# xbpeng/DeepTerrainRL

Measured on AMD Instinct MI355X. Metric: env-steps/sec (batched rollout) dog/slopes_mixed, higher is better.
Workload: dtype f64

## Files before the change

### deepterrainrl_amd/csrc/dtrl_kernel.h

```cpp
#pragma once
#include "dtrl_types.h"
#include <cmath>

#if defined(__HIPCC__)
#include <hip/hip_runtime.h>
#define DTRL_HD __host__ __device__
#define DTRL_HD_INLINE __host__ __device__ __forceinline__
#define DTRL_HD_NOINLINE __host__ __device__ __attribute__((noinline))
#else
#define DTRL_HD
#define DTRL_HD_INLINE inline
#define DTRL_HD_NOINLINE inline
#endif

#if defined(__HIP_DEVICE_COMPILE__)
#define LANES_BEGIN { const int lane = static_cast<int>(threadIdx.x);
#define LANES_END } ::dtrl::env_sync();
#else
#define LANES_BEGIN for (int lane = 0; lane < ::dtrl::kGroup; ++lane) {
#define LANES_END }
#endif

#if defined(__HIP_DEVICE_COMPILE__) && defined(DTRL_PROFILE)
#define PROF_T0() const unsigned long long prof_t0_ = __builtin_readcyclecounter()
// ... 91 lines not shown
	real px[kMaxL], py[kMaxL], cx[kMaxL], cy[kMaxL];
	real vpx[kMaxL], vpy[kMaxL], vcx[kMaxL], vcy[kMaxL];
	real fx[kMaxL], fy[kMaxL], fn[kMaxL];
	real mcx[kMaxL], mcy[kMaxL], Io[kMaxL];
	real sfs[3][kMaxL];
	union {
		struct { real bx[kMaxL], by[kMaxL], ux[kMaxL], uy[kMaxL], gx[kMaxL], gy[kMaxL]; };
		struct { real sm[kMaxL], smx[kMaxL], smy[kMaxL], sI[kMaxL]; };
	};
	real dinv[kMaxD];
	real b[kMaxD];
	real u[kMaxD];
	int32_t R, n_pts_active;
	int32_t row_kind[kMaxRows], row_link[kMaxRows];
	int8_t row_link2[kMaxRows];
	real row_x[kMaxRows], row_y[kMaxRows], row_dx[kMaxRows], row_dy[kMaxRows], row_tgt[kMaxRows];
	uint16_t row_id[kMaxRows];
	real wv[kMaxRows], rinv[kMaxRows];
	real dl;
	union {
		real Z[kMaxRows + 1][kZStride];
		struct {
			real z0_[kZStride];
			real basis[kMaxD][4];
			real tau_g[kMaxD];
			real kpv[kMaxD], kdv[kMaxD], kdm[kMaxD], perr[kMaxD], verr[kMaxD];
		};
	};
	real red[8];
	int32_t flag_update_action, flag_new_cycle, flag_misc;
	int32_t cost;
#if defined(DTRL_PROFILE)
	unsigned long long prof[kProfMax];
#endif
};
struct WSRef : WSBase {
	real H[kMaxD][kMaxD + 1];
	union {
		real A[kMaxRows][kMaxRows + 1];
		struct {
			real pt_x[kMaxPts], pt_y[kMaxPts], pt_depth[kMaxPts], pt_nx[kMaxPts], pt_ny[kMaxPts];
			int32_t pt_active[kMaxPts];
		};
	};
};
constexpr int kPackedA = kMaxRows * (kMaxRows + 1) / 2;
constexpr int kMassTab = kMaxL * (kMaxDepth + 2);
struct WSFast : WSBase {
	real Apk[kPackedA > kMassTab ? kPackedA : kMassTab];
};


DTRL_HD_INLINE real fmadd(real a, real b, real c) { return __builtin_fma(a, b, c); }
DTRL_HD_INLINE void sincos_r(real x, real* s, real* c)
{
#if defined(DTRL_REAL_F32)
	sincosf(x, s, c);
#else
	sincos(x, s, c);
#endif
}
#if defined(__HIP_DEVICE_COMPILE__)
typedef real v4r_t __attribute__((ext_vector_type(4)));
__device__ __forceinline__ v4r_t mfma_16x16x4(real a, real b, v4r_t acc)
{
#if defined(DTRL_REAL_F32)
	return __builtin_amdgcn_mfma_f32_16x16x4f32(a, b, acc, 0, 0, 0);
#else
	return __builtin_amdgcn_mfma_f64_16x16x4f64(a, b, acc, 0, 0, 0);
#endif
}
__device__ __forceinline__ constexpr int mfma_row(int r, int g)
{
#if defined(DTRL_REAL_F32)
	return 4 * g + r;
#else
	return 4 * r + g;
#endif
}
#endif
DTRL_HD_INLINE real fast_recip(real x)
{
#if defined(__HIP_DEVICE_COMPILE__)
	real r = __builtin_amdgcn_rcp(x);
	r = __builtin_fma(__builtin_fma(-x, r, 1.0), r, r);
	r = __builtin_fma(__builtin_fma(-x, r, 1.0), r, r);
	return r;
#else
	return 1.0 / x;
#endif
}
DTRL_HD_INLINE real fast_rsqrt(real x)
{
#if defined(__HIP_DEVICE_COMPILE__)
	real r = __builtin_amdgcn_rsq(x);
	const real hx = 0.5 * x;
	r = __builtin_fma(__builtin_fma(-hx * r, r, 0.5), r, r);
	r = __builtin_fma(__builtin_fma(-hx * r, r, 0.5), r, r);
	return r;
#else
	return 1.0 / sqrt(x);
#endif
}

DTRL_HD_INLINE real clamp_turn_rate(real v, int dof, real h)
{
	if (dof < 2) return v;
	const real vmax = kMaxTurnPerSubstep / h;
	return v > vmax ? vmax : (v < -vmax ? -vmax : v);
}
DTRL_HD inline real wrap_pi(real a)
{
	const real pi = 3.14159265358979323846, two_pi = 6.283185307179586476925286766559;
	real r = fmod(a + pi, two_pi);
	if (r < 0) r += two_pi;
	return r - pi;
}

DTRL_HD inline uint64_t rng_mix(uint64_t x)
{
	x += 0x9E3779B97F4A7C15ULL;
	x = (x ^ (x >> 30)) * 0xBF58476D1CE4E5B9ULL;
	x = (x ^ (x >> 27)) * 0x94D049BB133111EBULL;
	return x ^ (x >> 31);
}
struct Rng {
	uint64_t key; uint64_t* ctr;
	DTRL_HD real uniform() { uint64_t z = rng_mix(key + (*ctr) * 0xD1342543DE82EF95ULL); ++(*ctr); return static_cast<real>(z >> 11) * (1.0 / 9007199254740992.0); }
	DTRL_HD real uniform(real mn, real mx) { return mn + uniform() * (mx - mn); }
	DTRL_HD int rand_int(int mn, int mx) { if (mn == mx) return mn; int r = mn + static_cast<int>(uniform() * (mx - mn)); return r >= mx ? mx - 1 : r; }
	DTRL_HD bool flip() { return uniform() < 0.5; }
	DTRL_HD real normal(real mean, real stdev)
	{
		real u1 = 1.0 - uniform(), u2 = uniform();
		return mean + stdev * sqrt(-2.0 * log(u1)) * cos(6.283185307179586476925286766559 * u2);
	}
};
DTRL_HD inline Rng make_rng(const RunParams& rp, int env, uint64_t* ctr)
{
	Rng r; r.key = rng_mix(rp.rng_seed ^ rng_mix(static_cast<uint64_t>(rp.env_id_base + env))); r.ctr = ctr; return r;
}

struct GroundHdr { real mx0, o0, o1, sc0, sc1; int w0, w1; };
DTRL_HD_INLINE GroundHdr ground_header(const GroundRec& g)
{
	GroundHdr h;
	h.mx0 = g.max_x[0]; h.w0 = g.w[0]; h.w1 = g.w[1];
	h.o0 = g.origin_x[0]; h.o1 = g.origin_x[1]; h.sc0 = g.scale_x[0]; h.sc1 = g.scale_x[1];
	return h;
}
DTRL_HD_INLINE real sample_ground(const GroundRec& g, const GroundHdr& gh, real x, real* slope, int* oi, int* oj, int* oseg)
{
	const real mx0 = gh.mx0;
	const int w0 = gh.w0, w1 = gh.w1;
	const real o0 = gh.o0, o1 = gh.o1, sc0 = gh.sc0, sc1 = gh.sc1;
	const int seg = (x >= mx0) ? 1 : 0;
	const int w = seg ? w1 : w0;
	const real scale = seg ? sc1 : sc0;
	const real tol = 0.0001;
	real c = x - (seg ? o1 : o0);
	c /= scale;
	c += ((w - 1) * 0.5);
	if (c > -tol && c < w - 1 + tol) { c = c < 0.0 ? 0.0 : (c > w - 1.0 ? w - 1.0 : c); }
	c = !(c > 0.0) ? 0.0 : (c > w - 1.0 ? w - 1.0 : c);
	int i = static_cast<int>(c);
	int j = (i + 1 < w - 1) ? i + 1 : w - 1;
	real lerp = c - i;
	const real inv_run = fast_recip(scale * ((j - i) > 0 ? (j - i) : 1));
	real a = g.data[seg][i];
	real b = g.data[seg][j];
	if (slope) *slope = (j == i) ? 0.0 : (b - a) * inv_run;
	if (oi) *oi = i;
	if (oj) *oj = j;
	if (oseg) *oseg = seg;
	return (1 - lerp) * a + lerp * b;
}
DTRL_HD_INLINE real sample_ground(const GroundRec& g, real x, real* slope, int* oi, int* oj, int* oseg)
{
	const GroundHdr gh = ground_header(g);
	return sample_ground(g, gh, x, slope, oi, oj, oseg);
}

static_assert(kMaxDepth % 4 == 0, "path rows are read as 32-bit words");
template <class W>
DTRL_HD_INLINE uint32_t path_word(const W& ws, int j, int t)
{
#if defined(__HIP_DEVICE_COMPILE__)
	return reinterpret_cast<const uint32_t*>(&ws.M.path[j][0])[t];
#else
	uint32_t w; __builtin_memcpy(&w, &ws.M.path[j][4 * t], 4); return w;
#endif
}
template <class W>
DTRL_HD inline void kin_dyn_terms(W& ws)
{
	PROF_T0();
	LANES_BEGIN
	if (lane < ws.M.L) {
		const int j = lane;
		const int dep = ws.M.depth[j];
		real phi = 0, w = 0;
		const uint32_t pw[kMaxDepth / 4] = {path_word(ws, j, 0), path_word(ws, j, 1), path_word(ws, j, 2)};
#pragma unroll
		for (int k = 0; k < kMaxDepth; ++k) {
			const int a = (k <= dep) ? static_cast<int>((pw[k / 4] >> (8 * (k % 4))) & 0xffu) : 0;
			const real qa = ws.st.q[a + 2], wa = ws.st.qd[a + 2];
			const real on = (k <= dep) ? 1.0 : 0.0;
			phi = fmadd(qa, on, phi); w = fmadd(wa, on, w);
		}
		ws.phi[j] = phi; ws.w[j] = w;
		real s, c; sincos_r(phi, &s, &c);
		ws.cs[j] = c; ws.sn[j] = s;
	}
	LANES_END
	PROF_ADD(ws, kProfP1);
	LANES_BEGIN
	if (lane < ws.M.L) {
		const int j = lane;
		const int pa = ws.M.parent[j];
		real rx = 0, ry = 0, ux = 0, uy = 0, gx = 0, gy = 0;
		if (pa >= 0) {
			const real c = ws.cs[pa], s = ws.sn[pa], wp = ws.w[pa];
			rx = c * ws.M.attach[j][0] - s * ws.M.attach[j][1];
			ry = s * ws.M.attach[j][0] + c * ws.M.attach[j][1];
			ux = -(wp * ry); uy = wp * rx;
			const real w2 = wp * wp;
			gx = -(w2 * rx); gy = -(w2 * ry);
		}
// ... 1192 lines not shown
				else transition_state(ws, next);
			}
		} else {
			if ((state == stBackStance || state == stFrontStance) && ws.st.phase >= 1) advance = true;
			int trans_contact = (state == stExtend) ? jFinger : ((state == stGather) ? jToe : -1);
			if (trans_contact >= 0 && in_contact(ws, trans_contact)) advance = true;
			if (advance) {
				int next = ws.st.first_cycle ? stBackStance : ((state == stGather) ? stInvalid : state + 1);
				bool end_step = (next == stInvalid) || ws.st.first_cycle;
				if (end_step) do_update = 1; else transition_state(ws, next);
			}
		}
		ws.flag_update_action = do_update;
	}
	LANES_END
	PROF_ADD_SINCE(ws, kProfC_Fsm, pc_t); pc_t = PROF_NOW();
	if (__builtin_expect(ws.flag_update_action != 0, 0)) {
		PROF_T0();
		update_action<Ext>(ws, gm, rp, buf, g, env);
		PROF_ADD(ws, kProfAction);
		if (Ext) { if (ws.st.ext_park == kExtAwaiting) return; }
		LANES_BEGIN
		if (lane == 0) ws.st.first_cycle = 0;
		LANES_END
	}
	}
	LANES_BEGIN
	if (lane == 0) {
		real sx = 0, m = 0;
		for (int j = 0; j < L; ++j) { sx += ws.M.mass[j] * ws.vcx[j]; m += ws.M.mass[j]; }
		real com_vx = sx / m;
		if (raptor) {
			const int sh = stance_joint(ws, 0), st_toe = stance_joint(ws, 3);
			if (raptor_active_effector(ws, st_toe)) ws.st.pd_active_bits &= ~(1u << sh); else ws.st.pd_active_bits |= (1u << sh);
			real cv = ws.st.params[rmpCv], cd = ws.st.params[rmpCd];
			const bool first_half = ws.st.state == rstContact || ws.st.state == rstDown;
			cd = first_half ? 0 : cd; cv = first_half ? cv : 0;
			real com[2]; calc_com(ws, com);
			real d_theta = cd * (com[0] - (ws.st.q[0] + ws.cx[st_toe])) + cv * com_vx;
			ws.st.pd_target[swing_joint(ws, 0)] = ws.st.params[rmpMax + ws.st.state * rspMax + rspSwingHip] + d_theta;
		} else {
			const int joints[2] = {jHip, jShoulder}, effs[2] = {jToe, jFinger}, prm[2] = {spHip, spShoulder};
			for (int k = 0; k < 2; ++k) if (!in_contact(ws, effs[k])) {
				real default_theta = ws.st.params[mpMax + ws.st.state * spMax + prm[k]];
				ws.st.pd_target[joints[k]] = default_theta + com_vx * ws.st.params[mpCv];
			}
		}
	}
	LANES_END
	PROF_ADD_SINCE(ws, kProfC_Feedback, pc_t); pc_t = PROF_NOW();
	LANES_BEGIN
	if (lane < D) {
		const int i = lane;
		real kp = 0, kd = 0, kdm = 0, pe = 0, ve = 0;
		if (i >= 3) {
			const int j = i - 2;
			kdm = gm.kd[j];
			if ((ws.st.pd_active_bits >> j) & 1u) { kp = gm.kp[j]; kd = kdm; }
			real theta;
			if (gm.use_world[j]) {
				theta = wrap_pi(ws.phi[j] + gm.body_theta[j]);
				if (theta <= real(-2.0943951023931954923084289221863)) theta += real(6.283185307179586476925286766559);
			} else {
				theta = wrap_pi(ws.st.q[i] + gm.ref_theta[j]) - gm.ref_theta[j];
			}
			pe = ws.st.pd_target[j] - theta;
			ve = 0 - ws.st.qd[i];
		}
		ws.kpv[i] = kp; ws.kdv[i] = kd; ws.kdm[i] = kdm; ws.perr[i] = pe; ws.verr[i] = ve;
		ws.u[i] = kp * (pe - dt * ws.st.qd[i]) + kd * ve - quirk_bias(ws, i);
	}
	LANES_END
	PROF_ADD_SINCE(ws, kProfC_PdSetup, pc_t); pc_t = PROF_NOW();
	Path::pd_solve(ws, dt);
	PROF_ADD_SINCE(ws, kProfC_PdSolve, pc_t); pc_t = PROF_NOW();
	LANES_BEGIN
	if (lane < D) { const int i = lane; ws.tau_g[i] = 0; ws.st.tau_ctrl[i] = ws.kpv[i] * (ws.perr[i] - dt * ws.st.qd[i]) + ws.kdv[i] * (ws.verr[i] - dt * ws.u[i]); }
	LANES_END
	const int eff0 = raptor ? int(rRightToe) : int(jToe), eff1 = raptor ? int(rLeftToe) : int(jFinger);
	const bool sup0 = raptor ? raptor_active_effector(ws, eff0) : in_contact(ws, eff0);
	const bool sup1 = raptor ? raptor_active_effector(ws, eff1) : in_contact(ws, eff1);
	if (gm.enable_grav_comp && (sup0 || sup1)) {
		LANES_BEGIN
		if (lane < D) {
			const int d = lane;
			real tg;
			const real gy = kGravityY;
			if (d == 0) tg = 0;
			else if (d == 1) tg = -(ws.sm[0] * gy);
			else { const int l = d - 2; tg = -((ws.smx[l] - ws.sm[l] * ws.px[l]) * gy); }
			ws.tau_g[d] = tg;
			for (int e = 0; e < 2; ++e) {
				const int jid = e ? eff1 : eff0;
				real b0 = 0, b1 = 0;
				bool on_path = (d < 3) || ((ws.M.sub_mask[d - 2] >> jid) & 1u);
				if ((e ? sup1 : sup0) && on_path) {
					real pos[2]; effector_pos(ws, gm, jid, pos);
					const real fy[2] = {0, 1}, fxv[2] = {1, 0};
					b0 = jt_force(ws, d, pos, fy); b1 = jt_force(ws, d, pos, fxv);
				}
				ws.basis[d][e * 2 + 0] = b0; ws.basis[d][e * 2 + 1] = b1;
			}
		}
		LANES_END
		LANES_BEGIN
		if (lane == 0) {
			const real Wd[3] = {1, 1, 1}, Wr[3] = {0.0001, 0.0001, 1};
			real x[4];
			solve_ls4(ws.basis, ws.tau_g, raptor ? Wr : Wd, x);
			for (int k = 0; k < 4; ++k) ws.red[k] = x[k];
		}
		LANES_END
		LANES_BEGIN
		if (lane < D && (raptor || lane >= 3)) {
			const int d = lane;
			real s = 0; for (int k = 0; k < 4; ++k) s += ws.basis[d][k] * ws.red[k];
			ws.st.tau_ctrl[d] += ws.tau_g[d] - s;
		}
		LANES_END
	}
	PROF_ADD_SINCE(ws, kProfC_Grav, pc_t); pc_t = PROF_NOW();
	if (raptor) {
		LANES_BEGIN
// ... 363 lines not shown
```

### deepterrainrl_amd/csrc/dtrl_kernel_fast.h

```cpp
#pragma once
#include "dtrl_kernel.h"
#include "dtrl_topo.h"
#include <type_traits>

#if defined(__HIP_DEVICE_COMPILE__)

#if !DTRL_WAVE_SYNC
#error "dtrl_kernel_fast.h: the register-resident path is ONE wavefront per env by construction (v_readlane broadcasts, ballots, and LDS read-then-write sequences such as warm_match_fast() that rely on a wave's LDS operations completing in issue order). -DDTRL_WAVE_SYNC=0 builds the lane-phase reference path only (ADVICE r5)"
#endif

namespace dtrl {

__device__ __forceinline__ int lane_id() { return static_cast<int>(threadIdx.x); }
__device__ __forceinline__ int opaque_lane()
{
	int lane = static_cast<int>(threadIdx.x);
	asm volatile("" : "+v"(lane));
	return lane;
}
#if defined(DTRL_REAL_F32)
#define DTRL_VFMA "v_fma_f32"
#define DTRL_VMOV "v_mov_b32"
#else
#define DTRL_VFMA "v_fma_f64"
#define DTRL_VMOV "v_mov_b64"
#endif
__device__ __forceinline__ real bcast(real v, int src)
{
#if defined(DTRL_REAL_F32)
	return __int_as_float(__builtin_amdgcn_readlane(__float_as_int(v), src));
#else
	int lo = __builtin_amdgcn_readlane(__double2loint(v), src);
	int hi = __builtin_amdgcn_readlane(__double2hiint(v), src);
	return __hiloint2double(hi, lo);
#endif
}

template <int D>
__device__ __forceinline__ void mass_row(WSFast& ws, real (&h)[D])
{
	constexpr int Lk = D - 2;
	constexpr int kTab = Lk * (Lk + 5) / 2;
	constexpr int kFill = (kTab + 1) & ~1;
	static_assert(kFill <= static_cast<int>(sizeof(ws.Apk) / sizeof(real)), "mass table does not fit the packed-matrix storage");
	const int d = static_cast<int>(threadIdx.x);
	const int l = d >= 2 ? d - 2 : 0;
	const bool hinge = d >= 2 && d < D;
	real* T = ws.Apk;
	{
		struct alignas(2 * sizeof(real)) real2 { real x, y; };
		real2* T2 = reinterpret_cast<real2*>(T);
		const real2 z2 = {0.0, 0.0};
#pragma unroll
		for (int e = 0; e < (kFill / 2 + kGroup - 1) / kGroup; ++e) if (d + e * kGroup < kFill / 2) T2[d + e * kGroup] = z2;
	}
	env_sync();
	if (hinge) {
		const int base = l * (l + 5) / 2;
		const real m = ws.sm[l], mx = ws.smx[l], my = ws.smy[l];
		T[base] = -(my - m * ws.py[l]);
		T[base + 1] = (mx - m * ws.px[l]);
	}
	const int n_pairs = ws.M.n_pairs;
#pragma unroll 2
	for (int e = lane_id(); e < n_pairs; e += kGroup) {
		const int pl = ws.M.pair_l[e], pk = ws.M.pair_k[e];
		const int a = ws.M.path[pl][pk];
		const real m = ws.sm[pl], mx = ws.smx[pl], my = ws.smy[pl], I = ws.sI[pl];
		const real plx = ws.px[pl], ply = ws.py[pl];
		const real pax = ws.px[a], pay = ws.py[a];
		T[pl * (pl + 5) / 2 + 2 + a] = I - ((plx + pax) * mx + (ply + pay) * my) + m * (plx * pax + ply * pay);
	}
// ... 104 lines not shown
		fnma_lanes_lt<k>(z, h[k], zk);
	});
	return z;
}
template <class Topo>
constexpr int first_update_col(int i)
{
	for (int k = Topo::L + 1; k > i; --k) if (dof_coupled<Topo>(i, k)) return k;
	return 0;
}
template <class Topo, int kAhead = 1>
__device__ __forceinline__ void usolve_rows(WSFast& ws, int R)
{
	constexpr int D = Topo::L + 2;
	const int lane = static_cast<int>(threadIdx.x);
	if (lane > R) return;
	real* z = ws.Z[lane];
	const real* U = ws.Apk;
	real acc[D], u[D * (D - 1) / 2];
	auto fetch = [&](auto kc) {
		constexpr int k = decltype(kc)::value;
		static_for<0, k>([&](auto ic) {
			constexpr int i = decltype(ic)::value;
			if constexpr (dof_coupled<Topo>(i, k)) u[k * (k - 1) / 2 + i] = U[k * (k - 1) / 2 + i];
			if constexpr (first_update_col<Topo>(i) == k) acc[i] = z[i];
		});
		if constexpr (first_update_col<Topo>(k) == 0) acc[k] = z[k];
	};
	static_for_down<D - kAhead, D>(fetch);
	static_for_down<1, D>([&](auto kc) {
		constexpr int k = decltype(kc)::value;
		__builtin_amdgcn_sched_barrier(0);
		if constexpr (k - kAhead >= 1) fetch(std::integral_constant<int, k - kAhead>{});
		const real zk = acc[k];
		if constexpr (first_update_col<Topo>(k) != 0) z[k] = zk;
		static_for_down<0, k>([&](auto ic) {
			constexpr int i = decltype(ic)::value;
			if constexpr (dof_coupled<Topo>(i, k)) acc[i] = fmadd(-u[k * (k - 1) / 2 + i], zk, acc[i]);
		});
	});
	z[0] = acc[0];
}
template <int D>
__device__ __forceinline__ real utsolve_regs(const real (&h)[D], real u)
{
	static_for<0, D - 1>([&](auto kc) {
		constexpr int k = decltype(kc)::value;
		const real uk = bcast(u, k);
		fnma_lanes_ge<k + 1>(u, h[k], uk);
	});
	return u;
}

static_assert((kMaxPts + kGroup - 1) / kGroup == 3, "written for 3 sample points per lane");
struct ContactPts { PtVal p0, p1, p2; unsigned long long m0, m1, m2;  unsigned long long f0, f1, f2;  };
__device__ __forceinline__ unsigned link_field(unsigned long long m0, unsigned long long m1, unsigned long long m2, int link)
{
	const int b = link * kPtsPerLink, word = b >> 6, off = b & 63;
	unsigned long long lo = m0, hi = m1;
	if (word == 1) { lo = m1; hi = m2; }
	if (word == 2) { lo = m2; hi = 0ull; }
	unsigned long long bits = lo >> off;
	if (off + kPtsPerLink > 64) bits |= hi << (64 - off);
	return static_cast<unsigned>(bits & ((1ull << kPtsPerLink) - 1ull));
}
constexpr real kNoPoint = -1.0e30;
__device__ __noinline__ unsigned link_cap_drop_mask(WSFast& ws, real d0, real d1, real d2)
{
	const int lane = opaque_lane();
	const int npts = ws.M.L * kPtsPerLink;
	real* S = ws.Apk;
	if (lane < npts) S[lane] = d0;
	if (lane + kGroup < npts) S[lane + kGroup] = d1;
	if (lane + 2 * kGroup < npts) S[lane + 2 * kGroup] = d2;
	env_sync();
	auto over = [&](real d, int pt) -> unsigned {
		if (!(d > kNoPoint)) return 0u;
		const int base = (pt / kPtsPerLink) * kPtsPerLink;
		int rank = 0;
		for (int k = 0; k < kPtsPerLink; ++k) { const int o = base + k; const real od = S[o]; rank += (o != pt && (od > d || (od == d && o < pt))) ? 1 : 0; }
		return rank >= kMaxPtsPerLink ? 1u : 0u;
	};
	const unsigned m = over(d0, lane) | (over(d1, lane + kGroup) << 1) | (over(d2, lane + 2 * kGroup) << 2);
	env_sync();
	return m;
}
template <bool kFlags>
__device__ __forceinline__ ContactPts eval_points(WSFast& ws, const DevModel& gm, const GroundRec& g)
{
	const int lane = opaque_lane();
	const int npts = ws.M.L * kPtsPerLink;
	ContactPts c;
	PtVal z; z.x = 0; z.y = 0; z.depth = 0; z.nx = 0; z.ny = 0; z.active = 0; z.near = 0;
	c.p0 = z; c.p1 = z; c.p2 = z;
	if (lane < npts) c.p0 = contact_point_eval<kFlags>(ws, gm, g, lane);
	if (lane + kGroup < npts) c.p1 = contact_point_eval<kFlags>(ws, gm, g, lane + kGroup);
	if (lane + 2 * kGroup < npts) c.p2 = contact_point_eval<kFlags>(ws, gm, g, lane + 2 * kGroup);
	c.f0 = 0; c.f1 = 0; c.f2 = 0;
	if (kFlags) { c.f0 = __ballot(c.p0.near); c.f1 = __ballot(c.p1.near); c.f2 = __ballot(c.p2.near); }
	c.m0 = __ballot(c.p0.active); c.m1 = __ballot(c.p1.active); c.m2 = __ballot(c.p2.active);
	if ((c.m0 | c.m1 | c.m2) != 0ull) {
		const int many = (lane < ws.M.L) && __popc(link_field(c.m0, c.m1, c.m2, lane)) > kMaxPtsPerLink;
		if (__builtin_expect(__ballot(many) != 0ull, 0)) {
			const unsigned drop = link_cap_drop_mask(ws, c.p0.active ? c.p0.depth : kNoPoint, c.p1.active ? c.p1.depth : kNoPoint, c.p2.active ? c.p2.depth : kNoPoint);
			if (drop & 1u) c.p0.active = 0;
			if (drop & 2u) c.p1.active = 0;
			if (drop & 4u) c.p2.active = 0;
			c.m0 = __ballot(c.p0.active); c.m1 = __ballot(c.p1.active); c.m2 = __ballot(c.p2.active);
		}
	}
	return c;
}
__device__ __noinline__ unsigned row_cap_drop_mask(WSFast& ws, real d0, real d1, real d2, int cap)
{
	const int lane = opaque_lane();
	const int npts = ws.M.L * kPtsPerLink;
	real* S = ws.Apk;
	if (lane < npts) S[lane] = d0;
	if (lane + kGroup < npts) S[lane + kGroup] = d1;
	if (lane + 2 * kGroup < npts) S[lane + 2 * kGroup] = d2;
	env_sync();
	auto over = [&](real d, int pt) -> unsigned {
		if (!(d > kNoPoint)) return 0u;
		int rank = 0;
		for (int o = 0; o < npts; ++o) { const real od = S[o]; rank += (o != pt && (od > d || (od == d && o < pt))) ? 1 : 0; }
		return rank >= cap ? 1u : 0u;
	};
	const unsigned m = over(d0, lane) | (over(d1, lane + kGroup) << 1) | (over(d2, lane + 2 * kGroup) << 2);
	env_sync();
	return m;
}
__device__ __forceinline__ unsigned long long pairs_in_reach(const WSFast& ws)
{
	const int lane = static_cast<int>(threadIdx.x);
	return __ballot(lane < ws.M.n_cpairs && pair_in_reach(ws, lane));
}
constexpr int kPairCands = 2 * kPtsPerLink, kPairSlots = kGroup / kPairCands;
__device__ __noinline__ int append_pair_rows_fast(WSFast& ws, const DevModel& gm, int R, unsigned long long reach)
{
	const int lane = opaque_lane();
	const unsigned long long below = (lane == 0) ? 0ull : (~0ull >> (64 - lane));
	const int slot = lane / kPairCands, cand = lane - slot * kPairCands;
	while (reach != 0ull && R + 2 <= kMaxRows) {
		int mypr = -1;
#pragma unroll
		for (int sidx = 0; sidx < kPairSlots; ++sidx) {
			if (reach != 0ull) { const int pr = __ffsll(static_cast<long long>(reach)) - 1; reach &= reach - 1ull; if (slot == sidx) mypr = pr; }
		}
		int P = 0, Q = 0, k = 0;
		PairHit hit; hit.active = 0; hit.depth = 0; hit.x = 0; hit.y = 0; hit.nx = 0; hit.ny = 0;
		if (mypr >= 0) { pair_candidate(ws.M.cp_a[mypr], ws.M.cp_b[mypr], cand, &P, &Q, &k); hit = pair_point_eval(ws, gm, P, Q, k); }
		const unsigned long long am = __ballot(hit.active);
		if (am == 0ull) continue;
		int keep = hit.active;
		const int mine_cnt = __popcll((am >> (slot * kPairCands)) & ((1ull << kPairCands) - 1ull));
		if (__builtin_expect(__ballot(lane < kPairSlots * kPairCands && mine_cnt > kMaxPtsPerPair) != 0ull, 0)) {
			real* S = ws.Apk;
			S[lane] = hit.active ? hit.depth : -1.0;
			env_sync();
			if (hit.active) {
				int rank = 0;
				for (int o = 0; o < kPairCands; ++o) { const real od = S[slot * kPairCands + o]; rank += (o != cand && od > 0 && (od > hit.depth || (od == hit.depth && o < cand))) ? 1 : 0; }
				keep = rank < kMaxPtsPerPair;
			}
			env_sync();
		}
		const unsigned long long km = __ballot(keep);
		const int room = (kMaxRows - R) / 2;
		const int idx = __popcll(km & below);
		if (keep && idx < room) {
			const int Rw = R + 2 * idx;
			ws.row_kind[Rw] = 1; ws.row_link[Rw] = P; ws.row_link2[Rw] = static_cast<int8_t>(Q); ws.row_x[Rw] = hit.x; ws.row_y[Rw] = hit.y;
			ws.row_dx[Rw] = hit.nx; ws.row_dy[Rw] = hit.ny; ws.row_tgt[Rw] = 0;
			ws.row_id[Rw] = pair_row_id(mypr, cand, 0); ws.row_id[Rw + 1] = pair_row_id(mypr, cand, 1);
			ws.row_kind[Rw + 1] = 2; ws.row_link[Rw + 1] = P; ws.row_link2[Rw + 1] = static_cast<int8_t>(Q); ws.row_x[Rw + 1] = hit.x; ws.row_y[Rw + 1] = hit.y;
			ws.row_dx[Rw + 1] = hit.ny; ws.row_dy[Rw + 1] = -hit.nx; ws.row_tgt[Rw + 1] = 0;
		}
		int n = __popcll(km); if (n > room) n = room;
		R += 2 * n;
	}
	return R;
}
__device__ __forceinline__ void contact_bits_fast(WSFast& ws, unsigned long long m0, unsigned long long m1, unsigned long long m2)
{
	const int lane = static_cast<int>(threadIdx.x);
	int any = 0;
	if (lane < ws.M.L) any = link_field(m0, m1, m2, lane) != 0u;
	const unsigned long long lm = __ballot(any);
	if (lane == 0) ws.st.contact_bits = static_cast<uint32_t>(lm);
}
__device__ __forceinline__ void detect_contacts_fast(WSFast& ws, const DevModel& gm, const GroundRec& g)
{
	const ContactPts c = eval_points<true>(ws, gm, g);
	contact_bits_fast(ws, c.f0, c.f1, c.f2);
	env_sync();
}
__device__ __forceinline__ void emit_contact_rows(WSFast& ws, const PtVal& p, int pt, int rank, int cap, int R0, real inv_h)
{
	if (p.active && rank < cap) {
		const int R = R0 + 2 * rank;
		const int j = pt / kPtsPerLink;
		ws.row_kind[R] = 1; ws.row_link[R] = j; ws.row_link2[R] = -1; ws.row_x[R] = p.x; ws.row_y[R] = p.y;
		ws.row_dx[R] = p.nx; ws.row_dy[R] = p.ny; ws.row_tgt[R] = normal_row_target(p.depth, inv_h);
		ws.row_id[R] = ground_row_id(pt, 0); ws.row_id[R + 1] = ground_row_id(pt, 1);
		ws.row_kind[R + 1] = 2; ws.row_link[R + 1] = j; ws.row_link2[R + 1] = -1; ws.row_x[R + 1] = p.x; ws.row_y[R + 1] = p.y;
		ws.row_dx[R + 1] = p.ny; ws.row_dy[R + 1] = -p.nx; ws.row_tgt[R + 1] = 0;
	}
}
__device__ __forceinline__ void build_rows_fast(WSFast& ws, const DevModel& gm, const ContactPts& c_in, real h)
{
	ContactPts c = c_in;
	const int lane = opaque_lane();
	const unsigned long long below = (lane == 0) ? 0ull : (~0ull >> (64 - lane));
	const real inv_h = 1.0 / h;
	int lim = 0; real tgt = 0;
	if (lane >= 1 && lane < ws.M.L && !(ws.M.lim_lo[lane] > ws.M.lim_hi[lane])) {
		const real th = ws.st.q[lane + 2];
		if (th <= ws.M.lim_lo[lane] + kLimitSlop) { lim = 1; tgt = kLimitErp * fmax(ws.M.lim_lo[lane] - th, 0.0) * inv_h; }
		else if (th >= ws.M.lim_hi[lane] - kLimitSlop) { lim = -1; tgt = kLimitErp * fmax(th - ws.M.lim_hi[lane], 0.0) * inv_h; }
	}
	const unsigned long long ml = __ballot(lim != 0);
	const int rl = __popcll(ml & below);
	int R0 = __popcll(ml); if (R0 > kMaxRows) R0 = kMaxRows;
	if (lim != 0 && rl < kMaxRows) { ws.row_kind[rl] = 0; ws.row_link[rl] = lane; ws.row_link2[rl] = -1; ws.row_dx[rl] = lim; ws.row_tgt[rl] = tgt; ws.row_id[rl] = kNoRowId; }
	const int cap = (kMaxRows - R0) / 2;
	if (__builtin_expect(__popcll(c.m0) + __popcll(c.m1) + __popcll(c.m2) > cap, 0)) {
		const unsigned drop = row_cap_drop_mask(ws, c.p0.active ? c.p0.depth : kNoPoint, c.p1.active ? c.p1.depth : kNoPoint, c.p2.active ? c.p2.depth : kNoPoint, cap);
		if (drop & 1u) c.p0.active = 0;
		if (drop & 2u) c.p1.active = 0;
		if (drop & 4u) c.p2.active = 0;
		c.m0 = __ballot(c.p0.active); c.m1 = __ballot(c.p1.active); c.m2 = __ballot(c.p2.active);
	}
	const int n0 = __popcll(c.m0), n1 = __popcll(c.m1), n2 = __popcll(c.m2);
	emit_contact_rows(ws, c.p0, lane, __popcll(c.m0 & below), cap, R0, inv_h);
	emit_contact_rows(ws, c.p1, lane + kGroup, n0 + __popcll(c.m1 & below), cap, R0, inv_h);
	emit_contact_rows(ws, c.p2, lane + 2 * kGroup, n0 + n1 + __popcll(c.m2 & below), cap, R0, inv_h);
	int nc = n0 + n1 + n2; if (nc > cap) nc = cap;
	int R = R0 + 2 * nc;
	const unsigned long long reach = pairs_in_reach(ws);
	if (__builtin_expect(reach != 0ull, 0)) R = append_pair_rows_fast(ws, gm, R, reach);
	if (lane == 0) ws.R = R;
	env_sync();
}

template <int D>
__device__ __forceinline__ void build_delassus_fast(WSFast& ws, real h, real dinv_mine)
{
	const int lane = static_cast<int>(threadIdx.x);
	const int R = ws.R;
	const int n_ent = R * (R + 1) / 2;
	if (R < 16) {
		typedef v4r_t v4d_t;
		const int g = lane >> 4, c = lane & 15;
		real jv = 0;
		if (lane < R) {
			const int sw = lane;
			if (ws.row_kind[sw] == 0) jv = ws.row_dx[sw] * ws.st.qd[ws.row_link[sw] + 2];
			else jv = row_point_jv(ws, sw);
		}
		const int zrow = c <= R ? c : 0;
		v4d_t acc = {0, 0, 0, 0};
#pragma unroll
		for (int s4 = 0; s4 < (D + 3) / 4; ++s4) {
			const int k = 4 * s4 + g;
			const bool live = k < D;
			const real z = ws.Z[zrow][live ? k : 0], dk = ws.dinv[live ? k : 0];
			const real b = live ? z : 0.0;
			const real a = live ? z * dk : 0.0;
			acc = mfma_16x16x4(a, b, acc);
		}
#pragma unroll
		for (int r = 0; r < 4; ++r) {
			const int i = mfma_row(r, g);
			if (i < R && c <= i) ws.Apk[i * (i + 1) / 2 + c] = acc[r];
			if (i < R && c == R) ws.wv[i] = acc[r];
		}
		env_sync();
		if (lane < R) ws.wv[lane] = jv + h * ws.wv[lane] - ws.row_tgt[lane];
		env_sync();
		return;
	}
	const real* di = ws.dinv;
	auto entry_rows = [](int e, int& s, int& r) {
		s = static_cast<int>((sqrtf(8.0f * e + 1.0f) - 1.0f) * 0.5f);
		while (s * (s + 1) / 2 > e) --s;
		while ((s + 1) * (s + 2) / 2 <= e) ++s;
		r = e - s * (s + 1) / 2;
	};
	{
// ... 159 lines not shown
				pgs_rows_sweep<0, kPgsRegRows>(a, w, lam, rinv, tang, (static_cast<unsigned long long>(rows_hi) << 32) | rows_lo, lane, last);
			}
		}
		if (mine) ws.st.ws_lam[lane] = lam;
		env_sync();
		return;
	}
	const int tri = lane * (lane + 1) / 2;
	if (any_l0) for (int r = 0; r < R; ++r) if ((nz_l0 >> r) & 1ull) { const int mx = lane > r ? lane : r, mn = lane < r ? lane : r; w = fmadd(ws.Apk[mine ? mx * (mx + 1) / 2 + mn : 0], bcast(lam, r), w); }
	real a_nx = mine ? ws.Apk[tri] : 0.0;
	const unsigned long long actR = act & ((R < 64) ? ((1ull << R) - 1ull) : ~0ull);
	if (warm) {
		const unsigned long long pass0 = actR & ~tmask, pass1 = actR & tmask;
		for (int it = 0; it < kPgsIters; ++it) {
			for (int r = 0; r < R; ++r) {
				const real a_sr = a_nx;
				const int rn = (r + 1 < R) ? r + 1 : 0;
				{ const int mx = lane > rn ? lane : rn, mn = lane < rn ? lane : rn; a_nx = ws.Apk[mine ? mx * (mx + 1) / 2 + mn : 0]; }
				if (!((pass0 >> r) & 1ull)) continue;
				pgs_row_step<kPgsRowNormal>(w, lam, rinv, a_sr, r, lane, false, 0.0, 0.0);
			}
			const real ln = wave_shr1(lam);
			const real lim = kMu * ln;
			const unsigned long long rows = pass1 & __ballot(tang && ln > kHoldEps);
			for (int r = 0; r < R; ++r) {
				const real a_sr = a_nx;
				const int rn = (r + 1 < R) ? r + 1 : 0;
				{ const int mx = lane > rn ? lane : rn, mn = lane < rn ? lane : rn; a_nx = ws.Apk[mine ? mx * (mx + 1) / 2 + mn : 0]; }
				if (!((rows >> r) & 1ull)) continue;
				pgs_row_step<kPgsRowFriction>(w, lam, rinv, a_sr, r, lane, false, -lim, lim);
			}
		}
	} else {
		for (int it = 0; it < kPgsIters; ++it) {
			for (int r = 0; r < R; ++r) {
				const real a_sr = a_nx;
				const int rn = (r + 1 < R) ? r + 1 : 0;
				{ const int mx = lane > rn ? lane : rn, mn = lane < rn ? lane : rn; a_nx = ws.Apk[mine ? mx * (mx + 1) / 2 + mn : 0]; }
				if (!((act >> r) & 1ull)) continue;
				pgs_row_step<kPgsRowGeneric>(w, lam, rinv, a_sr, r, lane, tang, 0.0, 0.0);
			}
		}
	}
	if (mine) ws.st.ws_lam[lane] = lam;
	env_sync();
}

#if defined(DTRL_PROFILE)
__device__ __forceinline__ int prof_row_bucket(int R) { return R == 0 ? 0 : (R <= 6 ? 1 : (R <= 12 ? 2 : (R <= 18 ? 3 : 4))); }
#endif
template <class Topo>
struct FastPath {
	static constexpr int D = Topo::L + 2;
	static __device__ void substep(WSFast& ws, const DevModel& gm, const GroundRec& g, real h, bool kin_valid)
	{
		const int lane = static_cast<int>(threadIdx.x);
#if defined(DTRL_PROFILE)
		const unsigned long long prof_sub_t0 = __builtin_readcyclecounter();
#endif
		if (!kin_valid) { PROF_T0(); kin_dyn_terms(ws); PROF_ADD(ws, kProfFK); }
		const int rows_ready = kin_valid ? ws.n_pts_active : -1;
		if (rows_ready >= 0) {
			if (lane == 0) { ws.R = rows_ready; ws.n_pts_active = -1; }
			env_sync();
		} else {
			ContactPts cp;
			{ PROF_T0(); cp = eval_points<false>(ws, gm, g); PROF_ADD(ws, kProfDetect); }
			{ PROF_T0(); build_rows_fast(ws, gm, cp, h); PROF_ADD(ws, kProfRows); }
		}
		{ PROF_T0(); warm_match_fast(ws); PROF_ADD(ws, kProfRows); }
		real hrow[D];
		{ PROF_T0(); mass_row<D>(ws, hrow); PROF_ADD(ws, kProfMass); }
		real dinv;
		{ PROF_T0(); dinv = factorize_regs<Topo>(ws, hrow); PROF_ADD(ws, kProfFact); }
		const int R = ws.R;
		if (lane == 0) ws.cost += 8 + R;
		{
			PROF_T0();
			const bool hinge = lane >= 2 && lane < D;
			const real mypx = hinge ? ws.px[lane - 2] : 0.0, mypy = hinge ? ws.py[lane - 2] : 0.0;
			const uint32_t mysub = hinge ? ws.M.sub_mask[lane - 2] : 0u;
			real rhs0 = (lane < D) ? (ws.st.tau[lane] - ws.b[lane]) : 0.0;
			if (__builtin_expect(ws.st.pert_on != 0, 0)) { if (lane < D) rhs0 += perturb_gen_force(ws, lane); }
			auto rhs_of = [&](int r) -> real {
				if (r >= R) return rhs0;
				const int kind = ws.row_kind[r], link = ws.row_link[r];
				const real dx = ws.row_dx[r];
				if (kind == 0) return (lane == link + 2) ? dx : 0.0;
				const real dy = ws.row_dy[r], x = ws.row_x[r], y = ws.row_y[r];
				const int link2 = ws.row_link2[r];
				if (lane == 0) return link2 < 0 ? dx : 0.0;
				if (lane == 1) return link2 < 0 ? dy : 0.0;
				const int on = static_cast<int>((mysub >> link) & 1u) - (link2 < 0 ? 0 : static_cast<int>((mysub >> link2) & 1u));
				if (on == 0) return 0.0;
				const real jr = dx * (-(y - mypy)) + dy * (x - mypx);
				return on > 0 ? jr : -jr;
			};
			if (R < 1) {
				if (0 <= R) {
					const real z = usolve_regs<D>(hrow, rhs_of(0));
					if (lane < D) ws.Z[0][lane] = z;
				}
			} else {
				for (int r = 0; r <= R; ++r) { const real v = rhs_of(r); if (lane < D) ws.Z[r][lane] = v; }
				env_sync();
				usolve_rows<Topo>(ws, R);
			}
			if (lane < D) ws.dinv[lane] = dinv;
			env_sync();
			PROF_ADD(ws, kProfFsub);
#if defined(DTRL_PROFILE)
			PROF_ADD(ws, kProfFsubR0 + prof_row_bucket(R));
#endif
		}
		if (R > 0) {
			{ PROF_T0(); build_delassus_fast<D>(ws, h, dinv); PROF_ADD(ws, kProfDelassus); }
			{ PROF_T0(); pgs_solve_fast<Topo::kPgsRegRows>(ws); PROF_ADD(ws, kProfPgs); }
		}
		{
			PROF_T0();
			real u = 0;
			if (lane < D) {
				real s = h * ws.Z[R][lane];
				for (int r = 0; r < R; ++r) s = fmadd(ws.Z[r][lane], ws.st.ws_lam[r], s);
				u = s * dinv;
			}
			u = utsolve_regs<D>(hrow, u);
			if (lane < D) { const real v = clamp_turn_rate(ws.st.qd[lane] + u, lane, h); ws.st.qd[lane] = v; ws.st.q[lane] += h * v; }
			env_sync();
			PROF_ADD(ws, kProfFinish);
		}
#if defined(DTRL_PROFILE)
		if (threadIdx.x == 0) { ws.prof[kProfRowsSum] += R; ws.prof[kProfSubsteps] += 1; const int bk = prof_row_bucket(R); ws.prof[kProfR0 + bk] += 1; ws.prof[kProfT0 + bk] += __builtin_readcyclecounter() - prof_sub_t0; }
#endif
	}
	static __device__ void pd_solve(WSFast& ws, real dt)
	{
		const int lane = static_cast<int>(threadIdx.x);
		real hrow[D];
		mass_row<D>(ws, hrow);
		const real add = (lane < D) ? dt * ws.kdm[lane] : 0.0;
#pragma unroll
		for (int k = 0; k < D; ++k) if (lane == k) hrow[k] += add;
		const real dinv = factorize_regs<Topo>(ws, hrow);
		real z = (lane < D) ? ws.u[lane] : 0.0;
		z = usolve_regs<D>(hrow, z);
		real u = z * dinv;
		u = utsolve_regs<D>(hrow, u);
		env_sync();
		if (lane < D) ws.u[lane] = u;
		if (lane == 0) ws.R = 0;
		env_sync();
	}
	static __device__ void contacts(WSFast& ws, const DevModel& gm, const GroundRec& g, real h)
	{
		const ContactPts cp = eval_points<true>(ws, gm, g);
		contact_bits_fast(ws, cp.f0, cp.f1, cp.f2);
		build_rows_fast(ws, gm, cp, h);
		if (threadIdx.x == 0) ws.n_pts_active = ws.R;
		env_sync();
	}
};

}
#endif
```

Baseline: 20.00 million.

## Specialize contact point evaluation on link count and batch ground loads

Contact point evaluation is templated on the topology's link count, so the number of sample points per lane is a compile-time constant and unused point slots, ballots and cap-drop branches are removed. Per-point link data and ground cells are gathered in separate batched phases so the memory loads can be issued together before the arithmetic, with asm barriers pinning the loaded values. The PD setup is also rewritten branch-free using a clamped index and selects instead of divergent branches. The risks are higher register pressure from holding all points' values at once and some extra work on lanes that are not hinges.

```diff
diff --git a/deepterrainrl_amd/csrc/dtrl_kernel.h b/deepterrainrl_amd/csrc/dtrl_kernel.h
--- a/deepterrainrl_amd/csrc/dtrl_kernel.h
+++ b/deepterrainrl_amd/csrc/dtrl_kernel.h
@@ -167,6 +167,13 @@
 
 
 DTRL_HD_INLINE real fmadd(real a, real b, real c) { return __builtin_fma(a, b, c); }
+DTRL_HD_INLINE int opaque_index(int v)
+{
+#if defined(__HIP_DEVICE_COMPILE__)
+	asm volatile("" : "+v"(v));
+#endif
+	return v;
+}
 DTRL_HD_INLINE void sincos_r(real x, real* s, real* c)
 {
 #if defined(DTRL_REAL_F32)
@@ -264,7 +271,8 @@
 	h.o0 = g.origin_x[0]; h.o1 = g.origin_x[1]; h.sc0 = g.scale_x[0]; h.sc1 = g.scale_x[1];
 	return h;
 }
-DTRL_HD_INLINE real sample_ground(const GroundRec& g, const GroundHdr& gh, real x, real* slope, int* oi, int* oj, int* oseg)
+struct GroundCell { int seg, i, j; real lerp, inv_run; };
+DTRL_HD_INLINE GroundCell ground_cell(const GroundHdr& gh, real x)
 {
 	const real mx0 = gh.mx0;
 	const int w0 = gh.w0, w1 = gh.w1;
@@ -278,17 +286,28 @@
 	c += ((w - 1) * 0.5);
 	if (c > -tol && c < w - 1 + tol) { c = c < 0.0 ? 0.0 : (c > w - 1.0 ? w - 1.0 : c); }
 	c = !(c > 0.0) ? 0.0 : (c > w - 1.0 ? w - 1.0 : c);
-	int i = static_cast<int>(c);
-	int j = (i + 1 < w - 1) ? i + 1 : w - 1;
-	real lerp = c - i;
-	const real inv_run = fast_recip(scale * ((j - i) > 0 ? (j - i) : 1));
-	real a = g.data[seg][i];
-	real b = g.data[seg][j];
-	if (slope) *slope = (j == i) ? 0.0 : (b - a) * inv_run;
-	if (oi) *oi = i;
-	if (oj) *oj = j;
-	if (oseg) *oseg = seg;
-	return (1 - lerp) * a + lerp * b;
+	GroundCell k;
+	k.seg = seg;
+	k.i = static_cast<int>(c);
+	k.j = (k.i + 1 < w - 1) ? k.i + 1 : w - 1;
+	k.lerp = c - k.i;
+	k.inv_run = fast_recip(scale * ((k.j - k.i) > 0 ? (k.j - k.i) : 1));
+	return k;
+}
+DTRL_HD_INLINE real ground_height(const GroundCell& k, real a, real b, real* slope)
+{
+	if (slope) *slope = (k.j == k.i) ? 0.0 : (b - a) * k.inv_run;
+	return (1 - k.lerp) * a + k.lerp * b;
+}
+DTRL_HD_INLINE real sample_ground(const GroundRec& g, const GroundHdr& gh, real x, real* slope, int* oi, int* oj, int* oseg)
+{
+	const GroundCell k = ground_cell(gh, x);
+	real a = g.data[k.seg][k.i];
+	real b = g.data[k.seg][k.j];
+	if (oi) *oi = k.i;
+	if (oj) *oj = k.j;
+	if (oseg) *oseg = k.seg;
+	return ground_height(k, a, b, slope);
 }
 DTRL_HD_INLINE real sample_ground(const GroundRec& g, real x, real* slope, int* oi, int* oj, int* oseg)
 {
@@ -1587,23 +1606,20 @@
 	LANES_BEGIN
 	if (lane < D) {
 		const int i = lane;
-		real kp = 0, kd = 0, kdm = 0, pe = 0, ve = 0;
-		if (i >= 3) {
-			const int j = i - 2;
-			kdm = gm.kd[j];
-			if ((ws.st.pd_active_bits >> j) & 1u) { kp = gm.kp[j]; kd = kdm; }
-			real theta;
-			if (gm.use_world[j]) {
-				theta = wrap_pi(ws.phi[j] + gm.body_theta[j]);
-				if (theta <= real(-2.0943951023931954923084289221863)) theta += real(6.283185307179586476925286766559);
-			} else {
-				theta = wrap_pi(ws.st.q[i] + gm.ref_theta[j]) - gm.ref_theta[j];
-			}
-			pe = ws.st.pd_target[j] - theta;
-			ve = 0 - ws.st.qd[i];
-		}
+		const bool hinge = i >= 3;
+		const int j = opaque_index(hinge ? i - 2 : 1);
+		const real c_kd = gm.kd[j], c_kp = gm.kp[j], c_body = gm.body_theta[j], c_ref = gm.ref_theta[j];
+		const bool world = gm.use_world[j] != 0;
+		const real qd_i = ws.st.qd[i];
+		const bool active = ((ws.st.pd_active_bits >> j) & 1u) != 0;
+		const real kdm = hinge ? c_kd : 0;
+		const real kp = (hinge && active) ? c_kp : 0, kd = (hinge && active) ? c_kd : 0;
+		const real wr = wrap_pi(world ? ws.phi[j] + c_body : ws.st.q[i] + c_ref);
+		const real theta = world ? ((wr <= real(-2.0943951023931954923084289221863)) ? wr + real(6.283185307179586476925286766559) : wr) : wr - c_ref;
+		const real pe = hinge ? ws.st.pd_target[j] - theta : 0;
+		const real ve = hinge ? 0 - qd_i : 0;
 		ws.kpv[i] = kp; ws.kdv[i] = kd; ws.kdm[i] = kdm; ws.perr[i] = pe; ws.verr[i] = ve;
-		ws.u[i] = kp * (pe - dt * ws.st.qd[i]) + kd * ve - quirk_bias(ws, i);
+		ws.u[i] = kp * (pe - dt * qd_i) + kd * ve - quirk_bias(ws, i);
 	}
 	LANES_END
 	PROF_ADD_SINCE(ws, kProfC_PdSetup, pc_t); pc_t = PROF_NOW();
diff --git a/deepterrainrl_amd/csrc/dtrl_kernel_fast.h b/deepterrainrl_amd/csrc/dtrl_kernel_fast.h
--- a/deepterrainrl_amd/csrc/dtrl_kernel_fast.h
+++ b/deepterrainrl_amd/csrc/dtrl_kernel_fast.h
@@ -18,6 +18,8 @@
 	asm volatile("" : "+v"(lane));
 	return lane;
 }
+template <class T>
+__device__ __forceinline__ void pin_loaded(T& v) { asm volatile("" : "+v"(v)); }
 #if defined(DTRL_REAL_F32)
 #define DTRL_VFMA "v_fma_f32"
 #define DTRL_VMOV "v_mov_b32"
@@ -228,27 +230,30 @@
 	return u;
 }
 
-static_assert((kMaxPts + kGroup - 1) / kGroup == 3, "written for 3 sample points per lane");
+static_assert((kMaxPts + kGroup - 1) / kGroup == 3, "written for up to 3 sample points per lane");
+constexpr int pts_per_lane(int L) { return (L * kPtsPerLink + kGroup - 1) / kGroup; }
 struct ContactPts { PtVal p0, p1, p2; unsigned long long m0, m1, m2;  unsigned long long f0, f1, f2;  };
+template <int NP>
 __device__ __forceinline__ unsigned link_field(unsigned long long m0, unsigned long long m1, unsigned long long m2, int link)
 {
 	const int b = link * kPtsPerLink, word = b >> 6, off = b & 63;
-	unsigned long long lo = m0, hi = m1;
-	if (word == 1) { lo = m1; hi = m2; }
-	if (word == 2) { lo = m2; hi = 0ull; }
+	unsigned long long lo = m0, hi = NP > 1 ? m1 : 0ull;
+	if constexpr (NP > 1) if (word == 1) { lo = m1; hi = NP > 2 ? m2 : 0ull; }
+	if constexpr (NP > 2) if (word == 2) { lo = m2; hi = 0ull; }
 	unsigned long long bits = lo >> off;
 	if (off + kPtsPerLink > 64) bits |= hi << (64 - off);
 	return static_cast<unsigned>(bits & ((1ull << kPtsPerLink) - 1ull));
 }
 constexpr real kNoPoint = -1.0e30;
+template <int NP>
 __device__ __noinline__ unsigned link_cap_drop_mask(WSFast& ws, real d0, real d1, real d2)
 {
 	const int lane = opaque_lane();
 	const int npts = ws.M.L * kPtsPerLink;
 	real* S = ws.Apk;
 	if (lane < npts) S[lane] = d0;
-	if (lane + kGroup < npts) S[lane + kGroup] = d1;
-	if (lane + 2 * kGroup < npts) S[lane + 2 * kGroup] = d2;
+	if constexpr (NP > 1) if (lane + kGroup < npts) S[lane + kGroup] = d1;
+	if constexpr (NP > 2) if (lane + 2 * kGroup < npts) S[lane + 2 * kGroup] = d2;
 	env_sync();
 	auto over = [&](real d, int pt) -> unsigned {
 		if (!(d > kNoPoint)) return 0u;
@@ -257,44 +262,99 @@
 		for (int k = 0; k < kPtsPerLink; ++k) { const int o = base + k; const real od = S[o]; rank += (o != pt && (od > d || (od == d && o < pt))) ? 1 : 0; }
 		return rank >= kMaxPtsPerLink ? 1u : 0u;
 	};
-	const unsigned m = over(d0, lane) | (over(d1, lane + kGroup) << 1) | (over(d2, lane + 2 * kGroup) << 2);
+	unsigned m = over(d0, lane);
+	if constexpr (NP > 1) m |= over(d1, lane + kGroup) << 1;
+	if constexpr (NP > 2) m |= over(d2, lane + 2 * kGroup) << 2;
 	env_sync();
 	return m;
 }
-template <bool kFlags>
+template <int L, bool kFlags>
 __device__ __forceinline__ ContactPts eval_points(WSFast& ws, const DevModel& gm, const GroundRec& g)
 {
+	constexpr int NP = pts_per_lane(L), npts = L * kPtsPerLink;
 	const int lane = opaque_lane();
-	const int npts = ws.M.L * kPtsPerLink;
+	const GroundHdr gh = ground_header(g);
+	const real q0 = ws.st.q[0], q1 = ws.st.q[1];
+	const real tol = kFlags ? gm.contact_tol : real(0);
+	bool have[NP]; int col[NP]; real lx[NP], ly[NP], margin[NP], brk[NP], cs[NP], sn[NP], px[NP], py[NP];
+	static_for<0, NP>([&](auto ec) {
+		constexpr int e = decltype(ec)::value;
+		const int pt = lane + e * kGroup;
+		have[e] = (e + 1) * kGroup <= npts || pt < npts;
+		const int ptc = ((e + 1) * kGroup <= npts || pt < npts) ? pt : npts - 1;
+		const int j = ptc / kPtsPerLink;
+		col[e] = ws.M.col[j];
+		cs[e] = ws.cs[j]; sn[e] = ws.sn[j]; px[e] = ws.px[j]; py[e] = ws.py[j];
+		const real* lp = &gm.pt_ground[0][0][0] + 2 * ptc;
+		lx[e] = lp[0]; ly[e] = lp[1];
+		margin[e] = gm.link_margin[j]; brk[e] = gm.link_brk[j];
+	});
+	static_for<0, NP>([&](auto ec) {
+		constexpr int e = decltype(ec)::value;
+		pin_loaded(col[e]); pin_loaded(lx[e]); pin_loaded(ly[e]); pin_loaded(margin[e]); pin_loaded(brk[e]);
+	});
+	real x[NP], y[NP]; GroundCell cell[NP];
+	static_for<0, NP>([&](auto ec) {
+		constexpr int e = decltype(ec)::value;
+		x[e] = px[e] + cs[e] * lx[e] - sn[e] * ly[e];
+		y[e] = py[e] + sn[e] * lx[e] + cs[e] * ly[e];
+		cell[e] = ground_cell(gh, q0 + x[e]);
+	});
+	real ha[NP], hb[NP];
+	static_for<0, NP>([&](auto ec) {
+		constexpr int e = decltype(ec)::value;
+		ha[e] = g.data[cell[e].seg][cell[e].i];
+		hb[e] = g.data[cell[e].seg][cell[e].j];
+	});
+	PtVal r[3];
+	static_for<0, 3>([&](auto ec) {
+		constexpr int e = decltype(ec)::value;
+		r[e].x = 0; r[e].y = 0; r[e].depth = 0; r[e].nx = 0; r[e].ny = 0; r[e].active = 0; r[e].near = 0;
+		if constexpr (e < NP) {
+			real slope;
+			const real h = ground_height(cell[e], ha[e], hb[e], &slope);
+			const real gap = h - (q1 + y[e]);
+			const bool in_reach = kFlags || (gap + (margin[e] + brk[e]) * (1.0 + fabs(slope)) > 0);
+			const real inv = fast_rsqrt(1.0 + slope * slope);
+			const real depth = fmadd(gap, inv, margin[e]);
+			const bool live = have[e] & (col[e] != 0);
+			if (kFlags) r[e].near = (live & (depth >= -tol)) ? 1 : 0;
+			r[e].active = (live & in_reach & (depth > -brk[e])) ? 1 : 0;
+			r[e].nx = -slope * inv; r[e].ny = inv;
+			r[e].depth = depth;
+			r[e].x = x[e]; r[e].y = y[e];
+		}
+	});
 	ContactPts c;
-	PtVal z; z.x = 0; z.y = 0; z.depth = 0; z.nx = 0; z.ny = 0; z.active = 0; z.near = 0;
-	c.p0 = z; c.p1 = z; c.p2 = z;
-	if (lane < npts) c.p0 = contact_point_eval<kFlags>(ws, gm, g, lane);
-	if (lane + kGroup < npts) c.p1 = contact_point_eval<kFlags>(ws, gm, g, lane + kGroup);
-	if (lane + 2 * kGroup < npts) c.p2 = contact_point_eval<kFlags>(ws, gm, g, lane + 2 * kGroup);
+	c.p0 = r[0]; c.p1 = r[1]; c.p2 = r[2];
 	c.f0 = 0; c.f1 = 0; c.f2 = 0;
-	if (kFlags) { c.f0 = __ballot(c.p0.near); c.f1 = __ballot(c.p1.near); c.f2 = __ballot(c.p2.near); }
-	c.m0 = __ballot(c.p0.active); c.m1 = __ballot(c.p1.active); c.m2 = __ballot(c.p2.active);
+	if (kFlags) { c.f0 = __ballot(c.p0.near); if constexpr (NP > 1) c.f1 = __ballot(c.p1.near); if constexpr (NP > 2) c.f2 = __ballot(c.p2.near); }
+	c.m0 = __ballot(c.p0.active); c.m1 = 0; c.m2 = 0;
+	if constexpr (NP > 1) c.m1 = __ballot(c.p1.active);
+	if constexpr (NP > 2) c.m2 = __ballot(c.p2.active);
 	if ((c.m0 | c.m1 | c.m2) != 0ull) {
-		const int many = (lane < ws.M.L) && __popc(link_field(c.m0, c.m1, c.m2, lane)) > kMaxPtsPerLink;
+		const int many = (lane < L) && __popc(link_field<NP>(c.m0, c.m1, c.m2, lane)) > kMaxPtsPerLink;
 		if (__builtin_expect(__ballot(many) != 0ull, 0)) {
-			const unsigned drop = link_cap_drop_mask(ws, c.p0.active ? c.p0.depth : kNoPoint, c.p1.active ? c.p1.depth : kNoPoint, c.p2.active ? c.p2.depth : kNoPoint);
+			const unsigned drop = link_cap_drop_mask<NP>(ws, c.p0.active ? c.p0.depth : kNoPoint, (NP > 1 && c.p1.active) ? c.p1.depth : kNoPoint, (NP > 2 && c.p2.active) ? c.p2.depth : kNoPoint);
 			if (drop & 1u) c.p0.active = 0;
 			if (drop & 2u) c.p1.active = 0;
 			if (drop & 4u) c.p2.active = 0;
-			c.m0 = __ballot(c.p0.active); c.m1 = __ballot(c.p1.active); c.m2 = __ballot(c.p2.active);
+			c.m0 = __ballot(c.p0.active);
+			if constexpr (NP > 1) c.m1 = __ballot(c.p1.active);
+			if constexpr (NP > 2) c.m2 = __ballot(c.p2.active);
 		}
 	}
 	return c;
 }
+template <int NP>
 __device__ __noinline__ unsigned row_cap_drop_mask(WSFast& ws, real d0, real d1, real d2, int cap)
 {
 	const int lane = opaque_lane();
 	const int npts = ws.M.L * kPtsPerLink;
 	real* S = ws.Apk;
 	if (lane < npts) S[lane] = d0;
-	if (lane + kGroup < npts) S[lane + kGroup] = d1;
-	if (lane + 2 * kGroup < npts) S[lane + 2 * kGroup] = d2;
+	if constexpr (NP > 1) if (lane + kGroup < npts) S[lane + kGroup] = d1;
+	if constexpr (NP > 2) if (lane + 2 * kGroup < npts) S[lane + 2 * kGroup] = d2;
 	env_sync();
 	auto over = [&](real d, int pt) -> unsigned {
 		if (!(d > kNoPoint)) return 0u;
@@ -302,7 +362,9 @@
 		for (int o = 0; o < npts; ++o) { const real od = S[o]; rank += (o != pt && (od > d || (od == d && o < pt))) ? 1 : 0; }
 		return rank >= cap ? 1u : 0u;
 	};
-	const unsigned m = over(d0, lane) | (over(d1, lane + kGroup) << 1) | (over(d2, lane + 2 * kGroup) << 2);
+	unsigned m = over(d0, lane);
+	if constexpr (NP > 1) m |= over(d1, lane + kGroup) << 1;
+	if constexpr (NP > 2) m |= over(d2, lane + 2 * kGroup) << 2;
 	env_sync();
 	return m;
 }
@@ -357,19 +419,14 @@
 	}
 	return R;
 }
+template <int NP>
 __device__ __forceinline__ void contact_bits_fast(WSFast& ws, unsigned long long m0, unsigned long long m1, unsigned long long m2)
 {
 	const int lane = static_cast<int>(threadIdx.x);
 	int any = 0;
-	if (lane < ws.M.L) any = link_field(m0, m1, m2, lane) != 0u;
+	if (lane < ws.M.L) any = link_field<NP>(m0, m1, m2, lane) != 0u;
 	const unsigned long long lm = __ballot(any);
 	if (lane == 0) ws.st.contact_bits = static_cast<uint32_t>(lm);
-}
-__device__ __forceinline__ void detect_contacts_fast(WSFast& ws, const DevModel& gm, const GroundRec& g)
-{
-	const ContactPts c = eval_points<true>(ws, gm, g);
-	contact_bits_fast(ws, c.f0, c.f1, c.f2);
-	env_sync();
 }
 __device__ __forceinline__ void emit_contact_rows(WSFast& ws, const PtVal& p, int pt, int rank, int cap, int R0, real inv_h)
 {
@@ -383,6 +440,7 @@
 		ws.row_dx[R + 1] = p.ny; ws.row_dy[R + 1] = -p.nx; ws.row_tgt[R + 1] = 0;
 	}
 }
+template <int NP>
 __device__ __forceinline__ void build_rows_fast(WSFast& ws, const DevModel& gm, const ContactPts& c_in, real h)
 {
 	ContactPts c = c_in;
@@ -401,16 +459,18 @@
 	if (lim != 0 && rl < kMaxRows) { ws.row_kind[rl] = 0; ws.row_link[rl] = lane; ws.row_link2[rl] = -1; ws.row_dx[rl] = lim; ws.row_tgt[rl] = tgt; ws.row_id[rl] = kNoRowId; }
 	const int cap = (kMaxRows - R0) / 2;
 	if (__builtin_expect(__popcll(c.m0) + __popcll(c.m1) + __popcll(c.m2) > cap, 0)) {
-		const unsigned drop = row_cap_drop_mask(ws, c.p0.active ? c.p0.depth : kNoPoint, c.p1.active ? c.p1.depth : kNoPoint, c.p2.active ? c.p2.depth : kNoPoint, cap);
+		const unsigned drop = row_cap_drop_mask<NP>(ws, c.p0.active ? c.p0.depth : kNoPoint, (NP > 1 && c.p1.active) ? c.p1.depth : kNoPoint, (NP > 2 && c.p2.active) ? c.p2.depth : kNoPoint, cap);
 		if (drop & 1u) c.p0.active = 0;
 		if (drop & 2u) c.p1.active = 0;
 		if (drop & 4u) c.p2.active = 0;
-		c.m0 = __ballot(c.p0.active); c.m1 = __ballot(c.p1.active); c.m2 = __ballot(c.p2.active);
+		c.m0 = __ballot(c.p0.active);
+		if constexpr (NP > 1) c.m1 = __ballot(c.p1.active);
+		if constexpr (NP > 2) c.m2 = __ballot(c.p2.active);
 	}
 	const int n0 = __popcll(c.m0), n1 = __popcll(c.m1), n2 = __popcll(c.m2);
 	emit_contact_rows(ws, c.p0, lane, __popcll(c.m0 & below), cap, R0, inv_h);
-	emit_contact_rows(ws, c.p1, lane + kGroup, n0 + __popcll(c.m1 & below), cap, R0, inv_h);
-	emit_contact_rows(ws, c.p2, lane + 2 * kGroup, n0 + n1 + __popcll(c.m2 & below), cap, R0, inv_h);
+	if constexpr (NP > 1) emit_contact_rows(ws, c.p1, lane + kGroup, n0 + __popcll(c.m1 & below), cap, R0, inv_h);
+	if constexpr (NP > 2) emit_contact_rows(ws, c.p2, lane + 2 * kGroup, n0 + n1 + __popcll(c.m2 & below), cap, R0, inv_h);
 	int nc = n0 + n1 + n2; if (nc > cap) nc = cap;
 	int R = R0 + 2 * nc;
 	const unsigned long long reach = pairs_in_reach(ws);
@@ -676,6 +736,7 @@
 template <class Topo>
 struct FastPath {
 	static constexpr int D = Topo::L + 2;
+	static constexpr int NP = pts_per_lane(Topo::L);
 	static __device__ void substep(WSFast& ws, const DevModel& gm, const GroundRec& g, real h, bool kin_valid)
 	{
 		const int lane = static_cast<int>(threadIdx.x);
@@ -689,8 +750,8 @@
 			env_sync();
 		} else {
 			ContactPts cp;
-			{ PROF_T0(); cp = eval_points<false>(ws, gm, g); PROF_ADD(ws, kProfDetect); }
-			{ PROF_T0(); build_rows_fast(ws, gm, cp, h); PROF_ADD(ws, kProfRows); }
+			{ PROF_T0(); cp = eval_points<Topo::L, false>(ws, gm, g); PROF_ADD(ws, kProfDetect); }
+			{ PROF_T0(); build_rows_fast<NP>(ws, gm, cp, h); PROF_ADD(ws, kProfRows); }
 		}
 		{ PROF_T0(); warm_match_fast(ws); PROF_ADD(ws, kProfRows); }
 		real hrow[D];
@@ -778,9 +839,9 @@
 	}
 	static __device__ void contacts(WSFast& ws, const DevModel& gm, const GroundRec& g, real h)
 	{
-		const ContactPts cp = eval_points<true>(ws, gm, g);
-		contact_bits_fast(ws, cp.f0, cp.f1, cp.f2);
-		build_rows_fast(ws, gm, cp, h);
+		const ContactPts cp = eval_points<Topo::L, true>(ws, gm, g);
+		contact_bits_fast<NP>(ws, cp.f0, cp.f1, cp.f2);
+		build_rows_fast<NP>(ws, gm, cp, h);
 		if (threadIdx.x == 0) ws.n_pts_active = ws.R;
 		env_sync();
 	}
```

After: 20.50 million, median of 6. 2.5% higher.
